# hjsuh94/irs_mpc

Measured on AMD Instinct MI355X. Metric: rollouts*timesteps/s (randomized-smoothing pass) + iLQR-iters/s, higher is better.
Workload: dtype f32; 1 GPU; planar_hand quasi-dynamic contact, zero-order-B smoothing, step QP solved exactly (dual active-set method) -- the metric's config; T=50, N_per_gpu=10000, N_total=10000, mode=ZERO_ORDER_B, contact_solver=exact, samples=supplied, resident in HBM (f32), parallelism=samples sharded over 1 GPU(s), 1 all-reduce of (T,P) f64 per step

## Files before the change

### irs_mpc_amd/csrc/smooth_ug.hip

```cpp
#include "smooth_common.hpp"

namespace {

#ifndef IRS_UG_SWEEPS
#define IRS_UG_SWEEPS 6
#endif
#ifndef IRS_UG_FLIP_ALL
#define IRS_UG_FLIP_ALL 0
#endif
constexpr bool kUgFlipAll = IRS_UG_FLIP_ALL != 0;
#ifndef IRS_UG_PDAS
#define IRS_UG_PDAS (IRS_UG_FLIP_ALL ? 4 : 3)
#endif
#ifndef IRS_UG_PDAS_FLUSH
#define IRS_UG_PDAS_FLUSH (IRS_UG_FLIP_ALL ? 0 : 8)
#endif
#ifndef IRS_UG_BLOCK
#define IRS_UG_BLOCK 512
#endif
constexpr int kUgBlock = IRS_UG_BLOCK;
constexpr int kUgSweeps = IRS_UG_SWEEPS;
constexpr int kUgPdas = IRS_UG_PDAS;
constexpr int kUgPdasFlush = IRS_UG_PDAS_FLUSH;
#ifndef IRS_UG_STEP_COLUMNS
#define IRS_UG_STEP_COLUMNS 1
#endif
constexpr bool kUgStepColumns = IRS_UG_STEP_COLUMNS != 0;
#ifndef IRS_UG_TABLE_LDL
#define IRS_UG_TABLE_LDL 0
#endif
constexpr bool kUgTableLdl = IRS_UG_TABLE_LDL != 0;
constexpr int kUgTabH = 8, kUgTabTau = 40, kUgTabSet = 48, kUgTabX = 52;
constexpr int kUgTabStride = 116;
#ifndef IRS_UG_NOM_ROUNDS
#define IRS_UG_NOM_ROUNDS 2
#endif
constexpr int kUgNomRounds = IRS_UG_NOM_ROUNDS;
constexpr int kUgRing = 128;

template <class Model>
struct alignas(16) UgLds {
    static constexpr int NC = Model::NC, n = Model::NX, m = Model::NU;
    float tab[1 << NC][kUgTabStride];
    float W[NC][NC];
    float invw[NC];
    float Wd[NC];
    float r0[NC];
    float phi[NC];
    float C[m][NC];
    float JD[n][NC];
    float Jc[NC][n];
    float Dinv[n];
    float Db0[n];
    float DK[m];
    float q[n];
};

__device__ __forceinline__ float ug_uniform(float v) {
    return __int_as_float(__builtin_amdgcn_readfirstlane(__float_as_int(v)));
}

template <int NC>
struct UgUni {
    float W[NC * (NC + 1) / 2];
    float invw[NC];
    float r0[NC];
    __device__ __forceinline__ float w(int i, int j) const {
        return i <= j ? W[i * NC - i * (i - 1) / 2 + (j - i)] : W[j * NC - j * (j - 1) / 2 + (i - j)];
    }
};

template <class Model>
__device__ __forceinline__ unsigned ug_lookup_affine(const UgLds<Model>& S, unsigned a, const float* du, float tol,
                                                     float* v, float* tau) {
    constexpr int NC = Model::NC, m = Model::NU;
    static_assert(NC == 8 && m == 4, "table entries are 8 rows by 4 commands");
    const float4* e = reinterpret_cast<const float4*>(&S.tab[a][0]);
    float4 g4[kUgTabSet / 4];
#pragma unroll
    for (int c = 0; c < kUgTabSet / 4; ++c) g4[c] = e[c];
    const unsigned ap = __float_as_uint(S.tab[a][kUgTabSet]);
    tau[0] = g4[kUgTabTau / 4].x; tau[1] = g4[kUgTabTau / 4].y; tau[2] = g4[kUgTabTau / 4].z; tau[3] = g4[kUgTabTau / 4].w;
    tau[4] = g4[kUgTabTau / 4 + 1].x; tau[5] = g4[kUgTabTau / 4 + 1].y; tau[6] = g4[kUgTabTau / 4 + 1].z; tau[7] = g4[kUgTabTau / 4 + 1].w;
    v[0] = fmaf(tau[0], tol, g4[0].x); v[1] = fmaf(tau[1], tol, g4[0].y);
    v[2] = fmaf(tau[2], tol, g4[0].z); v[3] = fmaf(tau[3], tol, g4[0].w);
    v[4] = fmaf(tau[4], tol, g4[1].x); v[5] = fmaf(tau[5], tol, g4[1].y);
    v[6] = fmaf(tau[6], tol, g4[1].z); v[7] = fmaf(tau[7], tol, g4[1].w);
#pragma unroll
    for (int j = 0; j < m; ++j) {
        const float4 lo = g4[kUgTabH / 4 + 2 * j], hi = g4[kUgTabH / 4 + 2 * j + 1];
        v[0] = fmaf(lo.x, du[j], v[0]); v[1] = fmaf(lo.y, du[j], v[1]);
        v[2] = fmaf(lo.z, du[j], v[2]); v[3] = fmaf(lo.w, du[j], v[3]);
        v[4] = fmaf(hi.x, du[j], v[4]); v[5] = fmaf(hi.y, du[j], v[5]);
        v[6] = fmaf(hi.z, du[j], v[6]); v[7] = fmaf(hi.w, du[j], v[7]);
    }
    return ap;
}

template <class Model, bool UCOL>
__device__ __forceinline__ void ug_step_direction(const UgLds<Model>& S, unsigned a, int p, float* u, float* tau) {
    constexpr int NC = Model::NC;
    const float* e = &S.tab[a][0];
    const float4 t0 = *reinterpret_cast<const float4*>(e + kUgTabTau), t1 = *reinterpret_cast<const float4*>(e + kUgTabTau + 4);
    if constexpr (UCOL) {
        const float4 lo = *reinterpret_cast<const float4*>(e + kUgTabX + NC * p);
        const float4 hi = *reinterpret_cast<const float4*>(e + kUgTabX + NC * p + 4);
        u[0] = lo.x; u[1] = lo.y; u[2] = lo.z; u[3] = lo.w;
        u[4] = hi.x; u[5] = hi.y; u[6] = hi.z; u[7] = hi.w;
    } else {
        const float4 wlo = *reinterpret_cast<const float4*>(&S.W[p][0]);
        const float4 whi = *reinterpret_cast<const float4*>(&S.W[p][4]);
        const float4* x4 = reinterpret_cast<const float4*>(e + kUgTabX);
        float4 g4[2 * NC];
#pragma unroll
        for (int c = 0; c < 2 * NC; ++c) g4[c] = x4[c];
        const float wp[NC] = {wlo.x, wlo.y, wlo.z, wlo.w, whi.x, whi.y, whi.z, whi.w};
#pragma unroll
        for (int i = 0; i < NC; ++i) u[i] = 0.f;
#pragma unroll
        for (int c = 0; c < NC; ++c) {
            const float4 lo = g4[2 * c], hi = g4[2 * c + 1];
            u[0] = fmaf(lo.x, wp[c], u[0]); u[1] = fmaf(lo.y, wp[c], u[1]);
            u[2] = fmaf(lo.z, wp[c], u[2]); u[3] = fmaf(lo.w, wp[c], u[3]);
            u[4] = fmaf(hi.x, wp[c], u[4]); u[5] = fmaf(hi.y, wp[c], u[5]);
            u[6] = fmaf(hi.z, wp[c], u[6]); u[7] = fmaf(hi.w, wp[c], u[7]);
        }
    }
    tau[0] = t0.x; tau[1] = t0.y; tau[2] = t0.z; tau[3] = t0.w;
    tau[4] = t1.x; tau[5] = t1.y; tau[6] = t1.z; tau[7] = t1.w;
}

template <class Model>
__device__ __forceinline__ float ug_rhs(const UgUni<Model::NC>& U, const UgLds<Model>& S, const float* du, float* r) {
    constexpr int NC = Model::NC, m = Model::NU;
#pragma unroll
    for (int c = 0; c < NC; ++c) r[c] = U.r0[c];
#pragma unroll
    for (int j = 0; j < m; ++j) {
        const float4 lo = *reinterpret_cast<const float4*>(&S.C[j][0]);
        const float4 hi = *reinterpret_cast<const float4*>(&S.C[j][4]);
        r[0] = fmaf(lo.x, du[j], r[0]); r[1] = fmaf(lo.y, du[j], r[1]);
        r[2] = fmaf(lo.z, du[j], r[2]); r[3] = fmaf(lo.w, du[j], r[3]);
        r[4] = fmaf(hi.x, du[j], r[4]); r[5] = fmaf(hi.y, du[j], r[5]);
        r[6] = fmaf(hi.z, du[j], r[6]); r[7] = fmaf(hi.w, du[j], r[7]);
    }
    float scale = 1e-30f;
#pragma unroll
    for (int c = 0; c < NC; ++c) scale = fmaxf(scale, fabsf(r[c]));
    return 1e-6f * scale;
}

template <class Model, int CAP>
__device__ __forceinline__ void ug_pdas(const UgLds<Model>& S, const float* du, float tolv, unsigned& a, float* lam, bool& done) {
    constexpr int NC = Model::NC;
    static_assert(NC == 8, "the release key packs a row index into three mantissa bits");
    for (int it = 0; it < CAP; ++it) {
        float v[NC], tau[NC];
        const unsigned ap = ug_lookup_affine<Model>(S, a, du, tolv, v, tau);
        unsigned bad = 0u;
#pragma unroll
        for (int i = NC - 1; i >= 0; --i) bad = __builtin_amdgcn_alignbit(bad, __float_as_uint(v[i]), 31);
        unsigned next;
        if constexpr (kUgFlipAll) {
            next = ap ^ bad;
        } else {
            unsigned key = 0u;
#pragma unroll
            for (int i = 0; i < NC; ++i)
                key = max(key, (__float_as_uint(fmaf(tau[i], 3.0e38f, v[i])) & ~7u) | (unsigned)(7 - i));
            const unsigned worst = (bad & ap) != 0u ? (0x80u >> (key & 7u)) : 0u;
            next = (ap & ~worst) | (bad & ~ap);
        }
        if (!done) {
            if (bad == 0u) {
#pragma unroll
                for (int i = 0; i < NC; ++i) lam[i] = fmaf(-tau[i], v[i], v[i]);
                done = true;
            }
            a = next;
        }
        if (__all(done)) break;
    }
}

template <class Model>
__device__ __forceinline__ bool ug_try(const UgUni<Model::NC>& U, const UgLds<Model>& S, const float* r, const float* du,
                                       float tolv, float* lam, unsigned& a_out, int diag = 0) {
    constexpr int NC = Model::NC;
    float g[NC];
#pragma unroll
    for (int i = 0; i < NC; ++i) { lam[i] = 0.f; g[i] = r[i]; }
#pragma unroll 2
    for (int sw = 0; sw < ((diag & 64) ? 0 : kUgSweeps); ++sw) {
#pragma unroll
        for (int i = 0; i < NC; ++i) {
            const float nw = fmaxf(fmaf(-g[i], U.invw[i], lam[i]), 0.f);
            const float dl = nw - lam[i];
            lam[i] = nw;
#pragma unroll
            for (int j = 0; j < NC; ++j) g[j] = fmaf(U.w(j, i), dl, g[j]);
        }
    }
    unsigned a = 0u;
#pragma unroll
    for (int i = 0; i < NC; ++i) a |= (lam[i] > 0.f) ? (1u << i) : 0u;
    bool done = (diag & 32) != 0;
    ug_pdas<Model, kUgPdas>(S, du, tolv, a, lam, done);
    a_out = a;
    return done;
}

template <class Model, bool UCOL>
__device__ __forceinline__ void ug_full(const UgLds<Model>& S, const float* r, const float* du, float tolv, unsigned a,
                                        float* lam, int cap = 4 * Model::NC) {
    constexpr int NC = Model::NC;
    constexpr float kBig = 3.0e38f, piv_rel = 1e-5f;
    float g[NC];
    bool valid = false;
    for (int round = 0; round < 3; ++round) {
        if (__all(valid)) break;
        float v[NC], tau[NC];
        const unsigned ap = ug_lookup_affine<Model>(S, a, du, 0.f, v, tau);
        if (!valid) {
            unsigned negb = 0u;
#pragma unroll
            for (int i = 0; i < NC; ++i) {
                const bool in = tau[i] == 0.f;
                negb |= (in && !(v[i] > 0.f)) ? (1u << i) : 0u;
                lam[i] = in ? v[i] : 0.f;
                g[i] = in ? 0.f : v[i];
            }
            valid = negb == 0u;
            a = ap & ~negb;
        }
    }
    if (!valid) {
        a = 0u;
#pragma unroll
        for (int i = 0; i < NC; ++i) { lam[i] = 0.f; g[i] = r[i]; }
    }
    int p = -1;
    bool done = false;
    for (int it = 0; it < cap; ++it) {
        if (!done && p < 0) {
            float vmin = kBig;
            int c = 0;
#pragma unroll
            for (int i = 0; i < NC; ++i) {
                const float vv = ((a >> i) & 1u) ? kBig : g[i];
                if (vv < vmin) { vmin = vv; c = i; }
            }
            if (vmin >= -tolv) done = true;
            else p = c;
        }
        if (__all(done)) break;
        const int pp = (done || p < 0) ? 0 : p;
        float u[NC], tau[NC];
        ug_step_direction<Model, UCOL>(S, a, pp, u, tau);
        const float wpp = S.Wd[pp];
        float gp = 0.f, zp = 0.f;
#pragma unroll
        for (int i = 0; i < NC; ++i) {
            const bool isp = i == pp;
            gp = isp ? g[i] : gp;
            zp = isp ? u[i] : zp;
        }
        const bool full_ok = zp > piv_rel * wpp;
        const float t2 = full_ok ? -gp * irs_rcp_fast(zp) : kBig;
        float rho[NC], qv[NC];
        float t1 = kBig;
#pragma unroll
        for (int i = 0; i < NC; ++i) {
            rho[i] = fmaf(tau[i], u[i], -u[i]);
            qv[i] = rho[i] > 0.f ? lam[i] * irs_rcp_fast(rho[i]) : kBig;
            t1 = fminf(t1, qv[i]);
        }
        int kb = 0;
#pragma unroll
        for (int i = NC - 1; i >= 0; --i) kb = (qv[i] == t1) ? i : kb;
        const float tmin = fminf(t1, t2);
        if (!done && !(tmin < kBig)) done = true;
        const float tt = done ? 0.f : tmin;
#pragma unroll
        for (int i = 0; i < NC; ++i) {
            g[i] = fmaf(tt * tau[i], u[i], g[i]);
            lam[i] = fmaxf(fmaf(-tt, rho[i], lam[i]) + ((i == pp) ? tt : 0.f), 0.f);
        }
        if (!done) {
            const bool full = t2 <= t1;
            if (full) {
                a |= 1u << pp;
                p = -1;
            } else {
                a &= ~(1u << kb);
#pragma unroll
                for (int i = 0; i < NC; ++i) lam[i] = (i == kb) ? 0.f : lam[i];
            }
        }
    }
}

template <class Model, bool UCOL>
__device__ __forceinline__ void ug_build_entry(UgLds<Model>& S, unsigned a, int half) {
    constexpr int NC = Model::NC;
    constexpr float piv_rel = 1e-5f;
    float M_[NC][NC], inv[NC], W[NC][NC];
    bool act[NC];
#pragma unroll
    for (int i = 0; i < NC; ++i) {
        act[i] = ((a >> i) & 1u) != 0u;
#pragma unroll
        for (int j = 0; j < NC; ++j) W[i][j] = S.W[i][j];
#pragma unroll
        for (int j = 0; j <= i; ++j) M_[i][j] = W[i][j];
    }
    unsigned ap = 0u;
#pragma unroll
    for (int j = 0; j < NC; ++j) {
        const float dj = M_[j][j];
        const bool ok = act[j] && dj > piv_rel * W[j][j];
        act[j] = ok;
        ap |= ok ? (1u << j) : 0u;
        inv[j] = ok ? irs_rcp_fast(dj) : 0.f;
#pragma unroll
        for (int i = j + 1; i < NC; ++i) M_[j][i] = M_[i][j] * inv[j];
#pragma unroll
        for (int i = j + 1; i < NC; ++i)
#pragma unroll
            for (int k = j + 1; k <= i; ++k) M_[i][k] = M_[i][k] - M_[j][i] * M_[k][j];
    }
    float* e = &S.tab[a][0];
    constexpr int NAPP = 1 + Model::NU + NC, SHARE = (NAPP + 1) / 2;
    for (int qq = 0; qq < SHARE; ++qq) {
        const int q = half * SHARE + qq;
        if (q >= NAPP) break;
        const int c = q - (1 + Model::NU);
        float x[NC];
        if (UCOL || c < 0) {
            const float* src = q == 0 ? &S.r0[0] : (c < 0 ? &S.C[q - 1][0] : &S.W[c][0]);
            const float4 lo = *reinterpret_cast<const float4*>(src), hi = *reinterpret_cast<const float4*>(src + 4);
            x[0] = lo.x; x[1] = lo.y; x[2] = lo.z; x[3] = lo.w;
            x[4] = hi.x; x[5] = hi.y; x[6] = hi.z; x[7] = hi.w;
        } else {
#pragma unroll
            for (int i = 0; i < NC; ++i) x[i] = (i == c) ? 1.f : 0.f;
        }
        float y[NC];
#pragma unroll
        for (int j = 0; j < NC; ++j) {
            float v = act[j] ? -x[j] : 0.f;
#pragma unroll
            for (int k = 0; k < j; ++k) v = v - M_[k][j] * y[k];
            y[j] = v;
        }
#pragma unroll
        for (int j = NC - 1; j >= 0; --j) {
            float v = y[j] * inv[j];
#pragma unroll
            for (int i = j + 1; i < NC; ++i) v = v - M_[j][i] * y[i];
            y[j] = v;
        }
        float col[NC];
#pragma unroll
        for (int i = 0; i < NC; ++i) {
            float s = x[i];
#pragma unroll
            for (int j = 0; j < NC; ++j) s = fmaf(W[i][j], y[j], s);
            col[i] = act[i] ? y[i] : s;
        }
        float* dst = e + (c < 0 ? NC * q : kUgTabX + NC * c);
        *reinterpret_cast<float4*>(dst) = make_float4(col[0], col[1], col[2], col[3]);
        *reinterpret_cast<float4*>(dst + 4) = make_float4(col[4], col[5], col[6], col[7]);
    }
    if (half == 1) {
        *reinterpret_cast<float4*>(e + kUgTabTau) = make_float4(act[0] ? 0.f : 1.f, act[1] ? 0.f : 1.f, act[2] ? 0.f : 1.f, act[3] ? 0.f : 1.f);
        *reinterpret_cast<float4*>(e + kUgTabTau + 4) = make_float4(act[4] ? 0.f : 1.f, act[5] ? 0.f : 1.f, act[6] ? 0.f : 1.f, act[7] ? 0.f : 1.f);
        e[kUgTabSet] = __uint_as_float(ap);
    }
}

template <int NS>
struct UgTableau {
    float c[NS][8];
    unsigned set;
};

template <int P>
__device__ __forceinline__ float ug_bcast8(float v) {
    return __int_as_float(__builtin_amdgcn_ds_swizzle(__float_as_int(v), 0x18 | (P << 5)));
}

template <int P, int NS>
__device__ __forceinline__ void ug_pivot(UgTableau<NS>& R, bool want, float wpp) {
    constexpr float piv_rel = 1e-5f;
    constexpr int PS = (5 + P) >> 3, PL = (5 + P) & 7;
    float x[8];
#pragma unroll
    for (int i = 0; i < 8; ++i) x[i] = ug_bcast8<PL>(R.c[PS][i]);
    const float d = x[P];
    const bool ok = want && d > piv_rel * wpp;
    const float rinv = ok ? -irs_rcp_fast(d) : 0.f;
#pragma unroll
    for (int s = 0; s < NS; ++s) {
        const float rho = R.c[s][P] * rinv;
#pragma unroll
        for (int i = 0; i < 8; ++i)
            if (i != P) R.c[s][i] = fmaf(x[i], rho, R.c[s][i]);
        R.c[s][P] = ok ? rho : R.c[s][P];
    }
    R.set |= ok ? (1u << P) : 0u;
}

template <class Model, bool UCOL, int NS>
__device__ __forceinline__ void ug_emit_entry(UgLds<Model>& S, unsigned a, const UgTableau<NS>& R, int l) {
    float* e = &S.tab[a][0];
    auto put = [&](int off, const float* v) {
        *reinterpret_cast<float4*>(e + off) = make_float4(v[0], v[1], v[2], v[3]);
        *reinterpret_cast<float4*>(e + off + 4) = make_float4(v[4], v[5], v[6], v[7]);
    };
    if constexpr (UCOL) put(l < 5 ? 8 * l : kUgTabX + 8 * (l - 5), R.c[0]);
    else put(kUgTabX + 8 * l, R.c[2]);
    const float* v = UCOL ? R.c[1] : R.c[0];
    const int half = l == 6 ? 4 : 0;
    float4 q;
    q.x = l < 5 ? v[0] : (l == 7 ? __uint_as_float(R.set) : (((R.set >> (half + 0)) & 1u) ? 0.f : 1.f));
    q.y = l < 5 ? v[1] : (l == 7 ? 0.f : (((R.set >> (half + 1)) & 1u) ? 0.f : 1.f));
    q.z = l < 5 ? v[2] : (l == 7 ? 0.f : (((R.set >> (half + 2)) & 1u) ? 0.f : 1.f));
    q.w = l < 5 ? v[3] : (l == 7 ? 0.f : (((R.set >> (half + 3)) & 1u) ? 0.f : 1.f));
    const int off = l < 5 ? (UCOL ? kUgTabX + 8 * (l + 3) : 8 * l) : (l == 7 ? kUgTabSet : kUgTabTau + half);
    *reinterpret_cast<float4*>(e + off) = q;
    if (l < 5) *reinterpret_cast<float4*>(e + off + 4) = make_float4(v[4], v[5], v[6], v[7]);
}

template <class Model, bool UCOL>
__device__ __forceinline__ void ug_build_table(UgLds<Model>& S, int tid) {
    constexpr int NC = Model::NC, NS = UCOL ? 2 : 3, NW = kUgBlock / 64;
    static_assert(NC == 8 && Model::NU == 4, "an 8 x 13 tableau, eight lanes each");
    const int l = tid & 7;
    for (int w = __builtin_amdgcn_readfirstlane(tid >> 6); w < 8; w += NW) {
        const unsigned shared = (unsigned)(w ^ ((w & 4) ? 3 : 0));
        const unsigned g = ((unsigned)(tid >> 3) & 7u) | (shared << 3);
        UgTableau<NS> R;
        {
            const float* c0 = l == 0 ? &S.r0[0] : (l < 5 ? &S.C[l - 1][0] : &S.W[l - 5][0]);
            const float* c1 = &S.W[l < 5 ? l + 3 : 0][0];
            const float4 a0 = *reinterpret_cast<const float4*>(c0), a1 = *reinterpret_cast<const float4*>(c0 + 4);
            const float4 b0 = *reinterpret_cast<const float4*>(c1), b1 = *reinterpret_cast<const float4*>(c1 + 4);
            R.c[0][0] = a0.x; R.c[0][1] = a0.y; R.c[0][2] = a0.z; R.c[0][3] = a0.w;
            R.c[0][4] = a1.x; R.c[0][5] = a1.y; R.c[0][6] = a1.z; R.c[0][7] = a1.w;
            R.c[1][0] = b0.x; R.c[1][1] = b0.y; R.c[1][2] = b0.z; R.c[1][3] = b0.w;
            R.c[1][4] = b1.x; R.c[1][5] = b1.y; R.c[1][6] = b1.z; R.c[1][7] = b1.w;
            if constexpr (!UCOL) {
#pragma unroll
                for (int i = 0; i < NC; ++i) R.c[2][i] = (l == i) ? 1.f : 0.f;
            }
        }
        R.set = 0u;
        ug_pivot<0>(R, (g & 1u) != 0u, S.Wd[0]);
        ug_pivot<1>(R, (g & 2u) != 0u, S.Wd[1]);
        ug_pivot<2>(R, (g & 4u) != 0u, S.Wd[2]);
        if (shared & 1u) ug_pivot<3>(R, true, S.Wd[3]);
        if (shared & 2u) ug_pivot<4>(R, true, S.Wd[4]);
        if (shared & 4u) ug_pivot<5>(R, true, S.Wd[5]);
        UgTableau<NS> R6 = R, R7 = R;
        ug_pivot<6>(R6, true, S.Wd[6]);
        ug_pivot<7>(R7, true, S.Wd[7]);
        UgTableau<NS> R67 = R6;
        ug_pivot<7>(R67, true, S.Wd[7]);
        ug_emit_entry<Model, UCOL>(S, g, R, l);
        ug_emit_entry<Model, UCOL>(S, g | 64u, R6, l);
        ug_emit_entry<Model, UCOL>(S, g | 128u, R7, l);
        ug_emit_entry<Model, UCOL>(S, g | 192u, R67, l);
    }
}

struct UgNomLds {
    double J[8][7];
    double q[7], Dinv[7], b[7];
};

template <class Model, class Args>
__device__ __forceinline__ double ug_nominal_geometry(const Args& a, UgNomLds& L, int t, int lane) {
    constexpr int NC = Model::NC, n = Model::NX, m = Model::NU;
    double x64[n], u64[m], q[n], Dinv[n], b[n], J[NC][n], phi[NC];
#pragma unroll
    for (int i = 0; i < n; ++i) x64[i] = a.x_trj[(size_t)t * n + i];
#pragma unroll
    for (int j = 0; j < m; ++j) u64[j] = a.u_trj[(size_t)t * m + j];
    Model::template assemble<double>(a.p, x64, u64, q, Dinv, b, J, phi);
    if (lane == 0) {
#pragma unroll
        for (int c = 0; c < NC; ++c)
#pragma unroll
            for (int k = 0; k < n; ++k) L.J[c][k] = J[c][k];
#pragma unroll
        for (int k = 0; k < n; ++k) { L.q[k] = q[k]; L.Dinv[k] = Dinv[k]; L.b[k] = b[k]; }
    }
    double rr = 0.0;
#pragma unroll
    for (int c = 0; c < NC; ++c) {
        double s = phi[c];
#pragma unroll
        for (int k = 0; k < n; ++k) s -= J[c][k] * (b[k] * Dinv[k]);
        rr = (lane == c) ? s : rr;
    }
    wave_sync();
    return rr;
}

template <class Model, bool UCOL, class Args>
__device__ __forceinline__ void ug_nominal(const Args& a, const UgUni<Model::NC>& U, const UgLds<Model>& S,
                                           UgNomLds& L, double rr, int t, int lane) {
    constexpr int NC = Model::NC, n = Model::NX, m = Model::NU;
    static_assert(NC == 8 && n <= 8, "lane (i,k) = 8 i + k owns entry (i,k) of the 8 x 8 dual Hessian");
    float du0[m], r32[NC], lam32[NC];
#pragma unroll
    for (int j = 0; j < m; ++j) du0[j] = 0.f;
    const float tolv = ug_rhs<Model>(U, S, du0, r32);
    unsigned am = 0u;
    if (!ug_try<Model>(U, S, r32, du0, tolv, lam32, am)) ug_full<Model, UCOL>(S, r32, du0, tolv, am, lam32);
    unsigned set = 0u;
#pragma unroll
    for (int i = 0; i < NC; ++i) set |= (lam32[i] > 0.f) ? (1u << i) : 0u;
    set = (unsigned)__builtin_amdgcn_readfirstlane((int)set);
    {
        const int li = lane >> 3, lk = lane & 7;
        double w = 0.0;
#pragma unroll
        for (int kk = 0; kk < n; ++kk) w += L.J[li][kk] * L.Dinv[kk] * L.J[lk][kk];
        double scale = 1e-300;
#pragma unroll
        for (int c = 0; c < NC; ++c) scale = fmax(scale, fabs(__shfl(rr, c, 64)));
        const double tol64 = 1e-10 * scale;
        double lamd = 0.0;
        bool settled = false;
        for (int corr = 0; corr < 8 && !settled; ++corr) {
            double M = w, Lf = 0.0;
            unsigned eff = 0u;
            double invd[NC];
#pragma unroll
            for (int j = 0; j < NC; ++j) {
                const double dj = __shfl(M, 9 * j, 64), wjj = __shfl(w, 9 * j, 64);
                const bool ok = ((set >> j) & 1u) && dj > 1e-7 * wjj;
                eff |= ok ? (1u << j) : 0u;
                invd[j] = ok ? 1.0 / dj : 0.0;
                const double Mij = __shfl(M, 8 * li + j, 64), Mkj = __shfl(M, 8 * lk + j, 64);
                if (lk == j && li > j) Lf = Mij * invd[j];
                if (li > j && lk > j) M -= Mij * invd[j] * Mkj;
            }
            const bool mine = lane < NC && ((eff >> lane) & 1u);
            double y = mine ? -rr : 0.0;
#pragma unroll
            for (int j = 0; j < NC; ++j) {
                const double yj = __shfl(y, j, 64);
                const double Lij = __shfl(Lf, 8 * (lane & 7) + j, 64);
                if (lane < NC && lane > j) y -= Lij * yj;
            }
            double invme = 0.0;
#pragma unroll
            for (int j = 0; j < NC; ++j) invme = (lane == j) ? invd[j] : invme;
            y *= invme;
#pragma unroll
            for (int j = NC - 1; j >= 0; --j) {
                const double yj = __shfl(y, j, 64);
                const double Lji = __shfl(Lf, 8 * j + (lane & 7), 64);
                if (lane < j) y -= Lji * yj;
            }
            lamd = mine ? y : 0.0;
            double pr = w * __shfl(lamd, lk, 64);
            pr += __shfl_xor(pr, 1, 64);
            pr += __shfl_xor(pr, 2, 64);
            pr += __shfl_xor(pr, 4, 64);
            const double sl = rr + __shfl(pr, 8 * (lane & 7), 64);
            const bool neg = lane < NC && mine && !(lamd > 0.0);
            const bool viol = lane < NC && !mine && sl < -tol64;
            const unsigned negb = (unsigned)(__ballot(neg) & 0xffull), violb = (unsigned)(__ballot(viol) & 0xffull);
            if ((negb | violb) == 0u) settled = true;
            else set = (eff & ~negb) | violb;
        }
        double f = 0.0;
        if (settled) {
            double acc = 0.0;
#pragma unroll
            for (int c = 0; c < NC; ++c) acc += L.J[c][lane < n ? lane : 0] * __shfl(lamd, c, 64);
            if (lane < n) f = L.q[lane] + L.Dinv[lane] * (acc - L.b[lane]);
        } else if (lane < n) {
            float acc = -S.Db0[lane];
#pragma unroll
            for (int c = 0; c < NC; ++c) acc = fmaf(S.JD[lane][c], lam32[c], acc);
            f = (double)(S.q[lane] + acc);
        }
        if (lane < n)
            __hip_atomic_store(a.fnom + (size_t)t * n + Model::perm(lane), f, __ATOMIC_RELAXED, __HIP_MEMORY_SCOPE_AGENT);
    }
}

#ifdef IRS_UG_STAMPS
constexpr int kUgStampSlots = 12, kUgStampWgs = 2048;
__device__ unsigned long long ug_stamps[kUgStampWgs * kUgStampSlots];
#define UG_STAMP(slot)                                                                          \
    do {                                                                                        \
        if ((threadIdx.x & 63) == 0) {                                                          \
            const int wg_ = blockIdx.y * gridDim.x + blockIdx.x;                                \
            if (wg_ < kUgStampWgs && ((slot) < 8 ? threadIdx.x == 0 : true))                    \
                ug_stamps[wg_ * kUgStampSlots + (slot)] = __builtin_amdgcn_s_memtime();         \
        }                                                                                       \
    } while (0)
__device__ unsigned ug_counts[3];
#define UG_COUNT_DECL unsigned ug_cnt_[3] = {0u, 0u, 0u}
#define UG_COUNT(k, pred) ug_cnt_[k] += (unsigned)__popcll(__ballot(pred))
#define UG_COUNT_FLUSH                                                                          \
    do {                                                                                        \
        if ((threadIdx.x & 63) == 0)                                                            \
            for (int k_ = 0; k_ < 3; ++k_)                                                      \
                if (ug_cnt_[k_] != 0u) atomicAdd(&ug_counts[k_], ug_cnt_[k_]);                  \
    } while (0)
#else
#define UG_STAMP(slot) do {} while (0)
#define UG_COUNT_DECL do {} while (0)
#define UG_COUNT(k, pred) do {} while (0)
#define UG_COUNT_FLUSH do {} while (0)
#endif

template <class Model, bool UCOL>
__device__ __forceinline__ void ug_prologue(const ModelParams& p, const double* x, const double* u, bool build,
                                            UgLds<Model>& S, int tid) {
    constexpr int n = Model::NX, m = Model::NU, NC = Model::NC;
    const int lane = tid & 63, wave = tid >> 6;
    if (wave == 0) {
        float xb[n], ub[m], q[n], Dinv[n], b0[n], J[NC][n], phi[NC];
#pragma unroll
        for (int i = 0; i < n; ++i) xb[i] = (float)x[i];
#pragma unroll
        for (int j = 0; j < m; ++j) ub[j] = (float)u[j];
        Model::template assemble<float>(p, xb, ub, q, Dinv, b0, J, phi);
        if (lane == 0) {
#pragma unroll
            for (int i = 0; i < NC; ++i) {
                S.phi[i] = phi[i];
#pragma unroll
                for (int k = 0; k < n; ++k) S.Jc[i][k] = J[i][k];
            }
#pragma unroll
            for (int k = 0; k < n; ++k) { S.Db0[k] = b0[k] * Dinv[k]; S.q[k] = q[k]; S.Dinv[k] = Dinv[k]; }
#pragma unroll
            for (int j = 0; j < m; ++j) S.DK[j] = Dinv[Model::act(j)] * Model::template stiffness<float>(p, j);
        }
    }
    __syncthreads();
    if (tid < NC * NC) {
        const int i = tid / NC, j = tid % NC, hi = i > j ? i : j, lo = i > j ? j : i;
        float w = (S.Jc[hi][0] * S.Dinv[0]) * S.Jc[lo][0];
#pragma unroll
        for (int k = 1; k < n; ++k) w = w + (S.Jc[hi][k] * S.Dinv[k]) * S.Jc[lo][k];
        S.W[i][j] = w;
        if (i == j) {
            S.Wd[i] = w;
            S.invw[i] = (float)kContactPgsOmega * irs_rcp_fast(w);
        }
    } else if (tid < NC * NC + NC) {
        const int i = tid - NC * NC;
        float ri = S.phi[i];
#pragma unroll
        for (int k = 0; k < n; ++k) ri = ri - S.Jc[i][k] * S.Db0[k];
        S.r0[i] = ri;
    } else if (tid < 2 * NC * NC + NC) {
        const int e = tid - (NC * NC + NC), k = e / NC, c = e % NC;
        if (k < n) S.JD[k][c] = S.Jc[c][k] * S.Dinv[k];
    } else if (tid < 2 * NC * NC + NC + m * NC) {
        const int e = tid - (2 * NC * NC + NC), j = e / NC, c = e % NC;
        S.C[j][c] = (S.Jc[c][Model::act(j)] * S.Dinv[Model::act(j)]) * Model::template stiffness<float>(p, j);
    }
    __syncthreads();
    UG_STAMP(1);
    if (build) {
        if constexpr (kUgTableLdl) {
            for (int e = tid; e < 2 * (1 << NC); e += kUgBlock) ug_build_entry<Model, UCOL>(S, (unsigned)(e >> 1), e & 1);
        } else {
            ug_build_table<Model, UCOL>(S, tid);
        }
    }
    __syncthreads();
}

template <class Model, bool UCOL>
__global__ __launch_bounds__(kUgBlock) void ug_table_kernel(ModelParams p, const double* x, const double* u, float* out) {
    __shared__ UgLds<Model> S;
    const int tid = threadIdx.x;
    ug_prologue<Model, UCOL>(p, x, u, true, S, tid);
    constexpr int NE = 1 << Model::NC;
    for (int q = tid; q < NE * kUgTabStride; q += kUgBlock) {
        const int c = q % kUgTabStride;
        out[q] = (c > kUgTabSet && c < kUgTabX) ? 0.f : S.tab[q / kUgTabStride][c];
    }
}

template <class Model, int MODE, bool RNG, bool FUSE, bool BATCH>
__global__ __launch_bounds__(kUgBlock) void smooth_ug_kernel(SmoothArgs args, std::conditional_t<BATCH, SmoothBatch, SmoothSolo> bat) {
    using TR = SmoothTraits<Model, MODE>;
    constexpr int n = TR::n, m = TR::m, P = TR::P, NC = Model::NC;
    constexpr int BLOCK = kUgBlock, NW = BLOCK / 64;
    static_assert(TR::Z0 == n && NC == 8 && m == 4, "u-only smoothing of an 8-row contact model with 4 commands");
    static_assert(P < kBlock, "the hand-off's group reduction");
    constexpr int NG = m * (m + 1) / 2;
    constexpr int PI = TR::FIRST_B ? 1 : NG + m * NC + m;
    constexpr int PPI = irs_reduce_pad(TR::FIRST_B ? n * m : PI);
    constexpr int QE = m + 1;
    constexpr bool UCOL = !TR::FIRST_B && kUgStepColumns;
    __shared__ UgLds<Model> S;
    __shared__ UgNomLds nomL;
    __shared__ float ring_all[NW * kUgRing * QE];
    __shared__ float red[NW * (PPI > TR::PP ? PPI : TR::PP)];
    __shared__ float toti[PPI];
    __shared__ unsigned hist[TR::FIRST_B ? (1 << NC) : 1];
    __shared__ double red64[TR::NGRP * P];
    __shared__ double tot[P];
    __shared__ FinalizeLds<Model, MODE> fin;
    __shared__ int s_ticket;

    decltype(auto) a = smooth_row<Model, MODE>(args, bat, (int)blockIdx.y);
    const int t = smooth_row_t(a, (int)blockIdx.y), blk = blockIdx.x, tid = threadIdx.x;
    const int lane = tid & 63, wave = tid >> 6;

    UG_STAMP(0);
    const bool nominal_wave = blk == 0 && wave == NW - 1;
    double nom_r = 0.0;
    if (nominal_wave && !(a.diag & 2)) nom_r = ug_nominal_geometry<Model>(a, nomL, t, lane);
    if constexpr (TR::FIRST_B) {
        for (int q = tid; q < (1 << NC); q += BLOCK) hist[q] = 0u;
    }
    ug_prologue<Model, UCOL>(a.p, a.x_trj + (size_t)t * n, a.u_trj + (size_t)t * m, !(a.diag & 4), S, tid);

    UG_STAMP(2);
    UgUni<NC> U;
    {
        int q = 0;
#pragma unroll
        for (int i = 0; i < NC; ++i)
#pragma unroll
            for (int j = i; j < NC; ++j) U.W[q++] = S.W[i][j];
#pragma unroll
        for (int i = 0; i < NC; ++i) { U.invw[i] = S.invw[i]; U.r0[i] = S.r0[i]; }
    }

    float acc[PPI];
#pragma unroll
    for (int i = 0; i < PPI; ++i) acc[i] = 0.f;

    if (nominal_wave && !(a.diag & 2)) ug_nominal<Model, UCOL>(a, U, S, nomL, nom_r, t, lane);
    if (nominal_wave) UG_STAMP(8);
    UG_COUNT_DECL;
    if (!(a.diag & 8)) {
        const int V = a.nblk * NW;
        const int me = nominal_wave ? V - 1 : (blk == 0 ? wave : blk * NW - 1 + wave);
        const int nblocks = (a.N + 63) / 64;
        int round = nominal_wave ? kUgNomRounds : 0;
        auto block_of = [&](int k) { return k < kUgNomRounds ? k * (V - 1) + me : kUgNomRounds * (V - 1) + (k - kUgNomRounds) * V + me; };
        float* ring = ring_all + wave * (kUgRing * QE);
        int qhead = 0, qtail = 0;
        int bk = block_of(round);
        float du_next[m];
#pragma unroll
        for (int j = 0; j < m; ++j) du_next[j] = 0.f;
        auto request = [&](int block) {
            if constexpr (!RNG) {
                if (block < nblocks) {
                    const int sidx = block * 64 + lane;
                    const size_t row = (size_t)t * a.N + (sidx < a.N ? sidx : a.N - 1);
                    load_row<m>(a.du + row * m, du_next);
                }
            }
        };
        request(bk);
        while (true) {
            const bool fresh = bk < nblocks;
            const int pending = qtail - qhead;
            const bool flush = pending >= 64 || (!fresh && pending > 0);
            if (!fresh && !flush) break;
            float du[m], r[NC], lam[NC];
            bool on, fin_ = true;
            if (flush) {
                __builtin_amdgcn_fence(__ATOMIC_RELEASE, "wavefront");
                __builtin_amdgcn_wave_barrier();
                __builtin_amdgcn_fence(__ATOMIC_ACQUIRE, "wavefront");
                const int take = min(64, pending);
                on = lane < take;
                const int slot = (qhead + (on ? lane : 0)) & (kUgRing - 1);
#pragma unroll
                for (int j = 0; j < m; ++j) du[j] = ring[slot * QE + j];
                unsigned wm = __float_as_uint(ring[slot * QE + m]);
                const float tolv = ug_rhs<Model>(U, S, du, r);
                bool settled = false;
                if constexpr (kUgPdasFlush > 0) ug_pdas<Model, kUgPdasFlush>(S, du, tolv, wm, lam, settled);
                UG_COUNT(1, on && settled);
                UG_COUNT(2, on && !settled);
                if (!__all(settled)) {
                    float lf[NC];
                    ug_full<Model, UCOL>(S, r, du, tolv, wm, lf, (a.diag & 128) ? 8 : ((a.diag & 256) ? 12 : 4 * NC));
#pragma unroll
                    for (int i = 0; i < NC; ++i) lam[i] = settled ? lam[i] : lf[i];
                }
                qhead += take;
            } else {
                const int sidx = bk * 64 + lane;
                on = sidx < a.N;
                if constexpr (RNG) {
                    const unsigned long long gidx = a.sample_offset + (unsigned long long)sidx;
#pragma unroll
                    for (int j = n / 4; j < (n + m + 3) / 4; ++j) {
                        float g4[4];
                        philox_normal4(gidx, (unsigned)t, (unsigned)j, a.iter, a.seed, g4);
#pragma unroll
                        for (int c = 0; c < 4; ++c) {
                            const int idx = 4 * j + c;
                            if (idx >= n && idx < n + m) du[idx - n] = __fmul_rn(g4[c], a.std[idx]);
                        }
                    }
                } else {
#pragma unroll
                    for (int j = 0; j < m; ++j) du[j] = du_next[j];
                    request(block_of(round + 1));
                }
                const float tolv = ug_rhs<Model>(U, S, du, r);
                unsigned mask = 0u;
                fin_ = ug_try<Model>(U, S, r, du, tolv, lam, mask, a.diag);
                if (a.diag & 16) fin_ = true;
                const bool hard = on && !fin_;
                const unsigned long long bal = __ballot(hard);
                UG_COUNT(0, hard);
                if (hard) {
                    const int slot = (qtail + __popcll(bal & ((1ull << lane) - 1ull))) & (kUgRing - 1);
#pragma unroll
                    for (int j = 0; j < m; ++j) ring[slot * QE + j] = du[j];
                    ring[slot * QE + m] = __uint_as_float(mask);
                }
                qtail += __popcll(bal);
                bk = block_of(++round);
            }
            const bool use = on && fin_;
            bool nonfinite = false;
#pragma unroll
            for (int j = 0; j < m; ++j) nonfinite = nonfinite || irs_nonfinite_bits(du[j]);
            if constexpr (TR::FIRST_B) {
                unsigned I = 0u;
#pragma unroll
                for (int i = 0; i < NC; ++i) I |= (lam[i] * S.Wd[i] > (float)kContactActiveTol) ? (1u << i) : 0u;
                if (use) __hip_atomic_fetch_add(&hist[I], 1u, __ATOMIC_RELAXED, __HIP_MEMORY_SCOPE_WORKGROUP);
                if (on && nonfinite) acc[0] = irs_poison();
            } else {
                float zz[m];
#pragma unroll
                for (int j = 0; j < m; ++j) zz[j] = use ? du[j] : 0.f;
                int q = 0;
#pragma unroll
                for (int i = 0; i < m; ++i)
#pragma unroll
                    for (int j = i; j < m; ++j) { acc[q] = fmaf(zz[i], zz[j], acc[q]); ++q; }
#pragma unroll
                for (int i = 0; i < m; ++i)
#pragma unroll
                    for (int c = 0; c < NC; ++c) { acc[q] = fmaf(zz[i], lam[c], acc[q]); ++q; }
#pragma unroll
                for (int i = 0; i < m; ++i) { acc[q] += zz[i]; ++q; }
                if (on && nonfinite) acc[0] = irs_poison();
            }
        }
    }

    UG_STAMP(3);
    if (blk == 0 && wave == 1) UG_STAMP(9);
    if constexpr (TR::FIRST_B) {
        __syncthreads();
        unsigned poison_bits = __float_as_uint(acc[0]);
        asm volatile("" : "+v"(poison_bits));
#pragma unroll
        for (int i = 0; i < PPI; ++i) acc[i] = 0.f;
        for (int I = tid; I < (1 << NC); I += BLOCK) {
            const unsigned cnt = hist[I];
            if (cnt == 0u) continue;
            const float* e = &S.tab[I][0];
            const unsigned ap = __float_as_uint(e[kUgTabSet]);
            float Y[NC][m];
#pragma unroll
            for (int i = 0; i < NC; ++i) {
                const bool in = ((ap >> i) & 1u) != 0u;
#pragma unroll
                for (int c = 0; c < m; ++c) {
                    float s = 0.f;
#pragma unroll
                    for (int j = 0; j < NC; ++j) s = fmaf(e[kUgTabX + 8 * j + i], S.Jc[j][Model::act(c)], s);
                    Y[i][c] = in ? -s : 0.f;
                }
            }
#pragma unroll
            for (int k = 0; k < n; ++k)
#pragma unroll
                for (int c = 0; c < m; ++c) {
                    float s = 0.f;
#pragma unroll
                    for (int i = 0; i < NC; ++i) s = fmaf(S.Jc[i][k], Y[i][c], s);
                    const float Bkc = (k == Model::act(c) ? 1.f : 0.f) - S.Dinv[k] * s;
                    acc[Model::perm(k) * m + c] += (float)cnt * Bkc;
                }
        }
        if ((poison_bits & 0x7f800000u) == 0x7f800000u) acc[0] = irs_poison();
        block_reduce_lds<P, NW>(acc, red);
    } else {
        block_reduce_lds<PI, NW>(acc, red);
        __syncthreads();
        for (int q = tid; q < PI; q += BLOCK) {
            float s = red[q];
#pragma unroll
            for (int w = 1; w < NW; ++w) s += red[w * PPI + q];
            toti[q] = s;
        }
        __syncthreads();
        float out = 0.f;
        if (tid < P) {
            if (tid < NG) out = toti[tid];
            else if (tid < NG + m * n) {
                const int i = (tid - NG) / n, kext = (tid - NG) % n;
                int k = 0, jact = -1;
#pragma unroll
                for (int kk = 0; kk < n; ++kk) k = (Model::perm(kk) == kext) ? kk : k;
#pragma unroll
                for (int j = 0; j < m; ++j) jact = (Model::act(j) == k) ? j : jact;
                float s = -S.Db0[k] * toti[NG + m * NC + i];
                for (int c = 0; c < NC; ++c) s = fmaf(S.JD[k][c], toti[NG + i * NC + c], s);
                if (jact >= 0) {
                    const int lo = i < jact ? i : jact, hi = i < jact ? jact : i;
                    s = fmaf(S.DK[jact], toti[lo * m - lo * (lo - 1) / 2 + (hi - lo)], s);
                }
                out = s;
            } else {
                out = toti[NG + m * NC + (tid - NG - m * n)];
            }
        }
        __syncthreads();
        for (int q = tid; q < NW * TR::PP; q += BLOCK) red[q] = 0.f;
        __syncthreads();
        if (tid < P) red[tid] = out;
    }
    UG_STAMP(4);
    smooth_finish<Model, MODE, FUSE, BLOCK, true, std::remove_cv_t<std::remove_reference_t<decltype(a)>>>(a, red, red64, tot, fin, s_ticket, t, blk, tid, a.fnom + (size_t)t * n);
    UG_STAMP(5);
    UG_COUNT_FLUSH;
}

template <class Model, int MODE>
void ug_launch_m(const SmoothArgs& a, bool rng, bool fuse, hipStream_t st) {
    dim3 grid(a.nblk, a.T), block(kUgBlock);
    if (rng) {
        if (fuse) hipLaunchKernelGGL((smooth_ug_kernel<Model, MODE, true, true, false>), grid, block, 0, st, a, SmoothSolo{});
        else hipLaunchKernelGGL((smooth_ug_kernel<Model, MODE, true, false, false>), grid, block, 0, st, a, SmoothSolo{});
    } else {
        if (fuse) hipLaunchKernelGGL((smooth_ug_kernel<Model, MODE, false, true, false>), grid, block, 0, st, a, SmoothSolo{});
        else hipLaunchKernelGGL((smooth_ug_kernel<Model, MODE, false, false, false>), grid, block, 0, st, a, SmoothSolo{});
    }
}

template <class Model, int MODE>
void ug_launch_batch_m(const SmoothArgs& a, const SmoothBatch& bat, int B, hipStream_t st) {
    dim3 grid(a.nblk, B * a.T), block(kUgBlock);
    hipLaunchKernelGGL((smooth_ug_kernel<Model, MODE, true, true, true>), grid, block, 0, st, a, bat);
}

}

#ifdef IRS_UG_STAMPS
extern "C" int irs_debug_ug_stamps(unsigned long long* host_out, int n_wgs) {
    if (n_wgs > kUgStampWgs) n_wgs = kUgStampWgs;
    return (int)hipMemcpyFromSymbol(host_out, HIP_SYMBOL(ug_stamps), (size_t)n_wgs * kUgStampSlots * sizeof(unsigned long long));
}
extern "C" int irs_debug_ug_counts(unsigned* host_out3, int reset) {
    hipError_t e = hipMemcpyFromSymbol(host_out3, HIP_SYMBOL(ug_counts), 3 * sizeof(unsigned));
    const unsigned zero[3] = {0u, 0u, 0u};
    if (e == hipSuccess && reset) e = hipMemcpyToSymbol(HIP_SYMBOL(ug_counts), zero, sizeof(zero));
    return (int)e;
}
#endif

extern "C" int irs_debug_ug_table(int model, const double* params, const double* x, const double* u, int first_order,
                                  float* out_256x116) {
    using Model = PlanarHandExactModel;
    if (model != IRS_MODEL_PLANAR_HAND_EXACT) return IRS_ERR_UNSUPPORTED;
    IRS_CHECK_ARG(x && u && out_256x116, "null pointer");
    ModelParams p;
    int rc = irs_load_params(model, params, Model::NPARAMS, &p);
    if (rc != IRS_OK) return rc;
    constexpr size_t NOUT = (size_t)(1 << Model::NC) * kUgTabStride;
    double* dxu = nullptr;
    float* dout = nullptr;
    if (hipMalloc(&dxu, (Model::NX + Model::NU) * sizeof(double)) != hipSuccess) return IRS_ERR_HIP;
    if (hipMalloc(&dout, NOUT * sizeof(float)) != hipSuccess) { (void)hipFree(dxu); return IRS_ERR_HIP; }
    hipError_t e = hipMemcpy(dxu, x, Model::NX * sizeof(double), hipMemcpyHostToDevice);
    if (e == hipSuccess) e = hipMemcpy(dxu + Model::NX, u, Model::NU * sizeof(double), hipMemcpyHostToDevice);
    if (e == hipSuccess) {
        if (first_order) hipLaunchKernelGGL((ug_table_kernel<Model, false>), dim3(1), dim3(kUgBlock), 0, 0, p, dxu, dxu + Model::NX, dout);
        else hipLaunchKernelGGL((ug_table_kernel<Model, kUgStepColumns>), dim3(1), dim3(kUgBlock), 0, 0, p, dxu, dxu + Model::NX, dout);
        e = hipGetLastError();
    }
    if (e == hipSuccess) e = hipMemcpy(out_256x116, dout, NOUT * sizeof(float), hipMemcpyDeviceToHost);
    (void)hipFree(dxu);
    (void)hipFree(dout);
    return e == hipSuccess ? IRS_OK : IRS_ERR_HIP;
}

bool irs_smooth_ug_supported(int model, int mode) {
    const char* e = getenv("IRS_UG");
    if (e != nullptr && atoi(e) == 0) return false;
    return model == IRS_MODEL_PLANAR_HAND_EXACT && (mode == IRS_SMOOTH_ZERO_ORDER_B || mode == IRS_SMOOTH_FIRST_ORDER);
}

int irs_smooth_ug_nblk(int T, int N) {
    static int cus = 0;
    if (cus == 0) {
        hipDeviceProp_t prop;
        int dev = 0;
        cus = (hipGetDevice(&dev) == hipSuccess && hipGetDeviceProperties(&prop, dev) == hipSuccess)
                  ? prop.multiProcessorCount : 256;
        if (cus < 1) cus = 256;
    }
    const int nblocks = (N + 63) / 64, NW = kUgBlock / 64;
    int nb = cus / (T < 1 ? 1 : T);
    if (nb < 1) nb = 1;
    const int by_work = (nblocks + 1 + NW - 1) / NW;
    if (nb > by_work) nb = by_work;
    return nb < 1 ? 1 : nb;
}

int irs_smooth_ug_launch(int model, int mode, const SmoothArgs& a, bool rng, bool fuse, hipStream_t st) {
    if (model != IRS_MODEL_PLANAR_HAND_EXACT) return IRS_ERR_UNSUPPORTED;
    if (mode == IRS_SMOOTH_ZERO_ORDER_B) ug_launch_m<PlanarHandExactModel, IRS_SMOOTH_ZERO_ORDER_B>(a, rng, fuse, st);
    else if (mode == IRS_SMOOTH_FIRST_ORDER) ug_launch_m<PlanarHandExactModel, IRS_SMOOTH_FIRST_ORDER>(a, rng, fuse, st);
    else return IRS_ERR_UNSUPPORTED;
    return IRS_OK;
}

int irs_smooth_ug_launch_batch(int model, int mode, const SmoothArgs& a, const SmoothBatch& bat, int B, hipStream_t st) {
    if (model != IRS_MODEL_PLANAR_HAND_EXACT) return IRS_ERR_UNSUPPORTED;
    if (mode == IRS_SMOOTH_ZERO_ORDER_B) ug_launch_batch_m<PlanarHandExactModel, IRS_SMOOTH_ZERO_ORDER_B>(a, bat, B, st);
    else if (mode == IRS_SMOOTH_FIRST_ORDER) ug_launch_batch_m<PlanarHandExactModel, IRS_SMOOTH_FIRST_ORDER>(a, bat, B, st);
    else return IRS_ERR_UNSUPPORTED;
    return IRS_OK;
}
```

Before: 16.39 billion rollouts*timesteps/s.

## Spread planar-hand contact geometry across lanes and prefetch first sample block earlier

Replaces the serial per-thread assembly of the 8-contact planar hand geometry, in both the f32 prologue and the f64 nominal path, with a lane-parallel version. Each lane computes one contact row and one state entry, using DPP and shuffles to share values. It also hoists the first du sample-block load ahead of the prologue via an early callback, so the global load overlaps with geometry assembly and table construction. This cuts the serial prologue latency at the cost of hard-wiring the code to the planar hand model and keeping prefetched registers live across the prologue.

```diff
diff --git a/irs_mpc_amd/csrc/smooth_ug.hip b/irs_mpc_amd/csrc/smooth_ug.hip
--- a/irs_mpc_amd/csrc/smooth_ug.hip
+++ b/irs_mpc_amd/csrc/smooth_ug.hip
@@ -1,4 +1,5 @@
 #include "smooth_common.hpp"
+#include "ug_geometry.hpp"
 
 namespace {
 
@@ -482,30 +483,28 @@
 template <class Model, class Args>
 __device__ __forceinline__ double ug_nominal_geometry(const Args& a, UgNomLds& L, int t, int lane) {
     constexpr int NC = Model::NC, n = Model::NX, m = Model::NU;
-    double x64[n], u64[m], q[n], Dinv[n], b[n], J[NC][n], phi[NC];
+    static_assert(std::is_base_of<PlanarHandModel, Model>::value && NC == 8, "ug_hand_geometry is the planar hand's assembly");
+    double x64[n], u64[m];
 #pragma unroll
     for (int i = 0; i < n; ++i) x64[i] = a.x_trj[(size_t)t * n + i];
 #pragma unroll
     for (int j = 0; j < m; ++j) u64[j] = a.u_trj[(size_t)t * m + j];
-    Model::template assemble<double>(a.p, x64, u64, q, Dinv, b, J, phi);
-    if (lane == 0) {
-#pragma unroll
-        for (int c = 0; c < NC; ++c)
-#pragma unroll
-            for (int k = 0; k < n; ++k) L.J[c][k] = J[c][k];
-#pragma unroll
-        for (int k = 0; k < n; ++k) { L.q[k] = q[k]; L.Dinv[k] = Dinv[k]; L.b[k] = b[k]; }
-    }
-    double rr = 0.0;
-#pragma unroll
-    for (int c = 0; c < NC; ++c) {
-        double s = phi[c];
-#pragma unroll
-        for (int k = 0; k < n; ++k) s -= J[c][k] * (b[k] * Dinv[k]);
-        rr = (lane == c) ? s : rr;
-    }
+    UgHandLane<double> g;
+    ug_hand_geometry<double>(a.p, x64, u64, lane, g);
+    if (lane < NC) {
+#pragma unroll
+        for (int k = 0; k < n; ++k) L.J[lane][k] = g.J[k];
+    }
+    if (lane < n) { L.q[lane] = g.q; L.Dinv[lane] = g.Dinv; L.b[lane] = g.b; }
+    const double bD = g.b * g.Dinv;
+    const double bD1 = __shfl(bD, 1, 64), bD3 = __shfl(bD, 3, 64), bD4 = __shfl(bD, 4, 64), bD5 = __shfl(bD, 5, 64),
+                 bD6 = __shfl(bD, 6, 64);
+    const bool arm1 = (lane & 4) != 0;
+    double s = fma(-bD1, g.J[1], g.phi);
+    s = fma(-(arm1 ? bD5 : bD3), arm1 ? g.J[5] : g.J[3], s);
+    s = fma(-(arm1 ? bD6 : bD4), arm1 ? g.J[6] : g.J[4], s);
     wave_sync();
-    return rr;
+    return lane < NC ? s : 0.0;
 }
 
 template <class Model, bool UCOL, class Args>
@@ -622,30 +621,35 @@
 #define UG_COUNT_FLUSH do {} while (0)
 #endif
 
-template <class Model, bool UCOL>
+template <class Model, bool UCOL, class Early>
 __device__ __forceinline__ void ug_prologue(const ModelParams& p, const double* x, const double* u, bool build,
-                                            UgLds<Model>& S, int tid) {
+                                            UgLds<Model>& S, int tid, Early early) {
     constexpr int n = Model::NX, m = Model::NU, NC = Model::NC;
+    static_assert(std::is_base_of<PlanarHandModel, Model>::value && NC == 8, "ug_hand_geometry is the planar hand's assembly");
     const int lane = tid & 63, wave = tid >> 6;
     if (wave == 0) {
-        float xb[n], ub[m], q[n], Dinv[n], b0[n], J[NC][n], phi[NC];
-#pragma unroll
-        for (int i = 0; i < n; ++i) xb[i] = (float)x[i];
-#pragma unroll
-        for (int j = 0; j < m; ++j) ub[j] = (float)u[j];
-        Model::template assemble<float>(p, xb, ub, q, Dinv, b0, J, phi);
-        if (lane == 0) {
-#pragma unroll
-            for (int i = 0; i < NC; ++i) {
-                S.phi[i] = phi[i];
-#pragma unroll
-                for (int k = 0; k < n; ++k) S.Jc[i][k] = J[i][k];
-            }
-#pragma unroll
-            for (int k = 0; k < n; ++k) { S.Db0[k] = b0[k] * Dinv[k]; S.q[k] = q[k]; S.Dinv[k] = Dinv[k]; }
-#pragma unroll
-            for (int j = 0; j < m; ++j) S.DK[j] = Dinv[Model::act(j)] * Model::template stiffness<float>(p, j);
-        }
+        double xd[n], ud[m];
+#pragma unroll
+        for (int i = 0; i < n; ++i) xd[i] = x[i];
+#pragma unroll
+        for (int j = 0; j < m; ++j) ud[j] = u[j];
+        early();
+        float xb[n], ub[m];
+#pragma unroll
+        for (int i = 0; i < n; ++i) xb[i] = (float)xd[i];
+#pragma unroll
+        for (int j = 0; j < m; ++j) ub[j] = (float)ud[j];
+        UgHandLane<float> g;
+        ug_hand_geometry<float>(p, xb, ub, lane, g);
+        if (lane < NC) {
+            S.phi[lane] = g.phi;
+#pragma unroll
+            for (int k = 0; k < n; ++k) S.Jc[lane][k] = g.J[k];
+        }
+        if (lane < n) { S.Db0[lane] = g.b * g.Dinv; S.q[lane] = g.q; S.Dinv[lane] = g.Dinv; }
+        if (lane >= Model::act(0) && lane < Model::act(0) + m) S.DK[lane - Model::act(0)] = g.Dinv * g.kp;
+    } else {
+        early();
     }
     __syncthreads();
     if (tid < NC * NC) {
@@ -687,7 +691,7 @@
 __global__ __launch_bounds__(kUgBlock) void ug_table_kernel(ModelParams p, const double* x, const double* u, float* out) {
     __shared__ UgLds<Model> S;
     const int tid = threadIdx.x;
-    ug_prologue<Model, UCOL>(p, x, u, true, S, tid);
+    ug_prologue<Model, UCOL>(p, x, u, true, S, tid, [] {});
     constexpr int NE = 1 << Model::NC;
     for (int q = tid; q < NE * kUgTabStride; q += kUgBlock) {
         const int c = q % kUgTabStride;
@@ -726,10 +730,29 @@
     const bool nominal_wave = blk == 0 && wave == NW - 1;
     double nom_r = 0.0;
     if (nominal_wave && !(a.diag & 2)) nom_r = ug_nominal_geometry<Model>(a, nomL, t, lane);
+    if (nominal_wave) UG_STAMP(10);
     if constexpr (TR::FIRST_B) {
         for (int q = tid; q < (1 << NC); q += BLOCK) hist[q] = 0u;
     }
-    ug_prologue<Model, UCOL>(a.p, a.x_trj + (size_t)t * n, a.u_trj + (size_t)t * m, !(a.diag & 4), S, tid);
+    const int V = a.nblk * NW;
+    const int me = nominal_wave ? V - 1 : (blk == 0 ? wave : blk * NW - 1 + wave);
+    const int nblocks = (a.N + 63) / 64;
+    const int round0 = nominal_wave ? kUgNomRounds : 0;
+    auto block_of = [&](int k) { return k < kUgNomRounds ? k * (V - 1) + me : kUgNomRounds * (V - 1) + (k - kUgNomRounds) * V + me; };
+    float du_next[m];
+#pragma unroll
+    for (int j = 0; j < m; ++j) du_next[j] = 0.f;
+    auto request = [&](int block) {
+        if constexpr (!RNG) {
+            if (block < nblocks) {
+                const int sidx = block * 64 + lane;
+                const size_t row = (size_t)t * a.N + (sidx < a.N ? sidx : a.N - 1);
+                load_row<m>(a.du + row * m, du_next);
+            }
+        }
+    };
+    ug_prologue<Model, UCOL>(a.p, a.x_trj + (size_t)t * n, a.u_trj + (size_t)t * m, !(a.diag & 4), S, tid,
+                             [&] { if (!(a.diag & 8)) request(block_of(round0)); });
 
     UG_STAMP(2);
     UgUni<NC> U;
@@ -751,27 +774,10 @@
     if (nominal_wave) UG_STAMP(8);
     UG_COUNT_DECL;
     if (!(a.diag & 8)) {
-        const int V = a.nblk * NW;
-        const int me = nominal_wave ? V - 1 : (blk == 0 ? wave : blk * NW - 1 + wave);
-        const int nblocks = (a.N + 63) / 64;
-        int round = nominal_wave ? kUgNomRounds : 0;
-        auto block_of = [&](int k) { return k < kUgNomRounds ? k * (V - 1) + me : kUgNomRounds * (V - 1) + (k - kUgNomRounds) * V + me; };
+        int round = round0;
         float* ring = ring_all + wave * (kUgRing * QE);
         int qhead = 0, qtail = 0;
         int bk = block_of(round);
-        float du_next[m];
-#pragma unroll
-        for (int j = 0; j < m; ++j) du_next[j] = 0.f;
-        auto request = [&](int block) {
-            if constexpr (!RNG) {
-                if (block < nblocks) {
-                    const int sidx = block * 64 + lane;
-                    const size_t row = (size_t)t * a.N + (sidx < a.N ? sidx : a.N - 1);
-                    load_row<m>(a.du + row * m, du_next);
-                }
-            }
-        };
-        request(bk);
         while (true) {
             const bool fresh = bk < nblocks;
             const int pending = qtail - qhead;
@@ -864,6 +870,7 @@
                 for (int i = 0; i < m; ++i) { acc[q] += zz[i]; ++q; }
                 if (on && nonfinite) acc[0] = irs_poison();
             }
+            if (!flush && round == round0 + 1) UG_STAMP(6);
         }
     }
 
diff --git a/irs_mpc_amd/csrc/ug_geometry.hpp b/irs_mpc_amd/csrc/ug_geometry.hpp
--- /dev/null
+++ b/irs_mpc_amd/csrc/ug_geometry.hpp
@@ -0,0 +1,86 @@
+#pragma once
+
+#include "contact_models.hpp"
+
+__device__ __forceinline__ float ug_fma(float a, float b, float c) { return __builtin_fmaf(a, b, c); }
+__device__ __forceinline__ double ug_fma(double a, double b, double c) { return __builtin_fma(a, b, c); }
+
+__device__ __forceinline__ float ug_quad0(float v) {
+    return __int_as_float(__builtin_amdgcn_mov_dpp(__float_as_int(v), 0x00, 0xf, 0xf, true));
+}
+__device__ __forceinline__ double ug_quad0(double v) {
+    const int lo = __builtin_amdgcn_mov_dpp(__double2loint(v), 0x00, 0xf, 0xf, true);
+    const int hi = __builtin_amdgcn_mov_dpp(__double2hiint(v), 0x00, 0xf, 0xf, true);
+    return __hiloint2double(hi, lo);
+}
+
+template <typename T>
+struct UgHandLane {
+    T J[PlanarHandModel::NX];
+    T phi;
+    T q, Dinv, b;
+    T kp;
+};
+
+__device__ __forceinline__ float ug_rounded(float v) { asm volatile("" : "+v"(v)); return v; }
+__device__ __forceinline__ double ug_rounded(double v) { asm volatile("" : "+v"(v)); return v; }
+
+template <typename T>
+__device__ __forceinline__ void ug_hand_geometry(const ModelParams& p, const T* x_ext, const T* u, int lane, UgHandLane<T>& o) {
+    using M = PlanarHandModel;
+    const int r = lane & 7;
+    const bool arm1 = (r & 4) != 0, link1 = (r & 2) != 0, gen1 = (r & 1) != 0;
+    T q[M::NX];
+#pragma unroll
+    for (int k = 0; k < M::NX; ++k) q[k] = x_ext[M::perm(k)];
+    const T h = T(p.v[0]), g = T(p.v[1]), mass = T(p.v[2]), R = T(p.v[3]), mu = T(p.v[4]);
+    const T kp1 = T(p.v[5]), kp2 = T(p.v[6]), l1 = T(p.v[7]), l2 = T(p.v[8]), rl = T(p.v[9]), bx = T(p.v[10]);
+
+    const T a1 = arm1 ? q[5] : q[3] + T(3.14159265358979323846);
+    const T a12 = a1 + (arm1 ? q[6] : q[4]);
+    T dx, dy;
+    irs_sincos(link1 ? a12 : a1, dy, dx);
+    const T s1 = ug_quad0(dy), c1 = ug_quad0(dx);
+
+    const T base = arm1 ? bx : -bx;
+    const T lsel = link1 ? l1 : T(0);
+    const T L = link1 ? l2 : l1;
+    const T ax = ug_fma(c1, lsel, base), ay = ug_rounded(s1 * lsel);
+    const T rx = q[0] - ax, ry = ug_fma(-s1, lsel, q[1]);
+    T sp = ug_fma(ry, dy, rx * dx);
+    sp = sp < T(0) ? T(0) : (sp > L ? L : sp);
+    const T wx = ug_fma(dx, sp, ax), wy = ug_fma(dy, sp, ay);
+    T nx = q[0] - wx;
+    T ny = link1 ? q[1] - wy : ug_fma(-dy, sp, q[1]);
+    const T na = link1 ? nx : ny, nb = link1 ? ny : nx;
+    const T dist = irs_sqrt(ug_fma(na, na, nb * nb));
+    nx = nx / dist; ny = ny / dist;
+    const T gap = dist - (R + rl);
+    const T cx = ug_fma(nx, rl, wx), cy = ug_fma(ny, rl, wy);
+    const T r1x = cx - base, r1y = cy;
+    const T r2x = cx - ax, r2y = cy - ay;
+
+    const T sgn = gen1 ? -mu : mu;
+    const T ex = ug_fma(-ny, sgn, nx), ey = ug_fma(nx, sgn, ny);
+    const T j1 = ug_fma(r1y, ex, -(ey * r1x));
+    const T j2 = link1 ? ug_fma(ex, r2y, -(ey * r2x)) : T(0);
+    o.phi = gap;
+    o.J[0] = ex;
+    o.J[1] = ey;
+    o.J[2] = ug_fma(ny, ex, -(nx * ey)) * R;
+    o.J[3] = arm1 ? T(0) : j1;
+    o.J[4] = arm1 ? T(0) : j2;
+    o.J[5] = arm1 ? j1 : T(0);
+    o.J[6] = arm1 ? j2 : T(0);
+
+    const T inertia = T(0.5) * mass * R * R;
+    const T kp = (r & 1) ? kp1 : kp2;
+    const T qr = r == 0 ? q[0] : r == 1 ? q[1] : r == 2 ? q[2] : r == 3 ? q[3] : r == 4 ? q[4] : r == 5 ? q[5] : q[6];
+    const T ur = r == 3 ? u[0] : r == 4 ? u[1] : r == 5 ? u[2] : u[3];
+    const T num = r < 3 ? h * h : T(1);
+    const T den = r < 2 ? mass : r == 2 ? inertia : kp;
+    o.q = qr;
+    o.Dinv = num / den;
+    o.b = r < 3 ? (r == 1 ? mass * g : T(0)) : kp * (qr - ur);
+    o.kp = kp;
+}
```

New measurement: 17.30 billion rollouts*timesteps/s, median of 6. 5.6% higher.
